# rajasekarv/vega

Hardware: AMD Instinct MI355X
Metric: rows/sec (whole node) reduce_by_key i64→i64, 1e9 rows, 1/2/4/8 GPU (higher is better)
Workload: dtype int64; 1 GPU; C1: 1e9 (i64,i64) uniform keys in [0,2^63), reduce_by_key(sum), 256 partitions (BASELINE.json configs[1]); weak scaling: --rows per GPU; rows_per_gpu=1000000000, key_bits=63, nparts=256, distinct_keys_out=1000000000

## Files before the change

vega_amd/csrc/vega_api.hip:

```cpp
#include <hip/hip_runtime.h>
#include <rccl/rccl.h>
#include <cmath>
#include <cstdio>
#include <cstring>
#include <map>
#include <string>
#include <vector>

#include "../../include/vega_common.h"
#include "../../include/vega_gpu.h"
#include "vega_internal.h"

using namespace vega;

struct RddImpl {
    uint64_t n = 0;
    int vtype = 0;
    int64_t *d_k = nullptr;
    void *d_v = nullptr;
    void *d_v2 = nullptr;
    uint64_t alloc_rows = 0;
    uint32_t nparts = 1;
    bool sorted = false;
    bool grouped = false;
// ... 1532 lines not shown
                          int64_t *out_k, int64_t *out_va, int64_t *out_vb,
                          uint64_t cap, uint64_t *h_nout, void *d_ws, size_t ws_bytes) {
    Ws ws(d_ws, ws_bytes);
    hipError_t e = join_sorted((hipStream_t)stream, ak, av, na, bk, bv, nb, order_mode,
                               out_k, out_va, out_vb, cap, h_nout, ws);
    return e == hipSuccess ? VEGA_OK : VEGA_ERR_HIP;
}

size_t vega_dev_select_ws_bytes(uint64_t num, uint64_t cand_cap) {
    return select_ws_bytes(num, cand_cap);
}

int vega_dev_select_k_i64(void *stream, const int64_t *keys, const int64_t *vals, uint64_t n,
                          uint64_t num, int descending, uint64_t cand_cap,
                          int64_t *out_k, int64_t *out_v, uint64_t *h_nout, int *h_passes,
                          void *d_ws, size_t ws_bytes) {
    if (!h_nout || !h_passes) return VEGA_ERR_INVALID;
    *h_nout = 0;
    *h_passes = 0;
    if (n >= (1ULL << 32)) return VEGA_ERR_UNSUPPORTED;
    const uint64_t m = num < n ? num : n;
    if (!m) return VEGA_OK;
    if (!keys || !vals || !out_k || !out_v) return VEGA_ERR_INVALID;
    if (!d_ws || ws_bytes < select_ws_bytes(m, cand_cap)) return VEGA_ERR_CAP;
    Ws ws(d_ws, ws_bytes);
    const char *msg = "";
    hipError_t e = select_k((hipStream_t)stream, keys, vals, n, m, descending != 0, cand_cap,
                            out_k, out_v, h_nout, h_passes, ws, &msg);
    if (e == hipSuccess) e = hipStreamSynchronize((hipStream_t)stream);
    if (e != hipSuccess && *msg) fprintf(stderr, "vega_dev_select_k_i64: %s\n", msg);
    if (e == hipErrorNotSupported) return VEGA_ERR_UNSUPPORTED;
    return e == hipSuccess ? VEGA_OK : (e == hipErrorOutOfMemory ? VEGA_ERR_CAP : VEGA_ERR_HIP);
}

int vega_dev_reduce_pairs(void *stream, const int64_t *keys, const void *vals, uint64_t n, int op,
                          int64_t *h_out_k, void *h_out_v, void *d_ws, size_t ws_bytes) {
    if (!n || !keys || !vals || !h_out_k || !h_out_v) return VEGA_ERR_INVALID;
    if (op != VEGA_OP_SUM_I64 && op != VEGA_OP_SUM_F64 && op != VEGA_OP_MIN_I64 &&
        op != VEGA_OP_MAX_I64)
        return VEGA_ERR_INVALID;
    Ws ws(d_ws, ws_bytes);
    hipError_t e = col_reduce((hipStream_t)stream, keys, vals, n, op, h_out_k, h_out_v, ws);
    if (e == hipErrorNotSupported) return VEGA_ERR_UNSUPPORTED;
    return e == hipSuccess ? VEGA_OK : (e == hipErrorOutOfMemory ? VEGA_ERR_CAP : VEGA_ERR_HIP);
}

int vega_dev_sample(void *stream, const int64_t *keys, const void *vals, uint64_t n,
                    int with_replacement, double fraction, uint64_t seed, uint64_t start,
                    int64_t *out_k, void *out_v, uint64_t cap, uint64_t *h_nout,
                    void *d_ws, size_t ws_bytes) {
    if (!h_nout) return VEGA_ERR_INVALID;
    *h_nout = 0;
    SampleSpec sp;
    int rc = sample_spec(with_replacement, fraction, seed, start, &sp, nullptr, 0);
    if (rc) return rc;
    if (n >= (1ULL << 32)) return VEGA_ERR_UNSUPPORTED;
    if (!n) return VEGA_OK;
    if (!keys || !vals) return VEGA_ERR_INVALID;
    if (!d_ws || ws_bytes < sample_ws_bytes(n)) return VEGA_ERR_NOMEM;
    Ws ws(d_ws, ws_bytes);
    SamplePlan pl;
    uint64_t total = 0;
    hipError_t e = sample_count((hipStream_t)stream, n, sp, &pl, &total, ws);
    if (e != hipSuccess) return hip_rc(e);
    *h_nout = total;
    if (total >= (1ULL << 32)) return VEGA_ERR_UNSUPPORTED;
    if (total > cap) return VEGA_ERR_CAP;
    if (!total) return VEGA_OK;
    if (!out_k || !out_v) return VEGA_ERR_INVALID;
    e = sample_emit((hipStream_t)stream, (const uint64_t *)keys, (const uint64_t *)vals, n, sp,
                    pl, (uint64_t *)out_k, (uint64_t *)out_v);
    if (e == hipSuccess) e = hipStreamSynchronize((hipStream_t)stream);
    return hip_rc(e);
}

int vega_phase_prof_read(unsigned long long out[8], int reset) {
    unsigned long long *b = vega::phase_prof_buf();
    if (!b) return VEGA_ERR_UNSUPPORTED;
    if (hipMemcpy(out, b, 8 * 8, hipMemcpyDeviceToHost) != hipSuccess) return VEGA_ERR_HIP;
    if (reset) (void)hipMemset(b, 0, 8 * 8);
    return VEGA_OK;
}

int vega_dev_checksum_pairs(void *stream, const int64_t *keys, const int64_t *vals,
                            uint64_t n, uint64_t *h_sum, void *d_ws, size_t ws_bytes) {
    Ws ws(d_ws, ws_bytes);
    return checksum_pairs((hipStream_t)stream, keys, vals, n, h_sum, ws) == hipSuccess
               ? VEGA_OK : VEGA_ERR_HIP;
}

}
```

vega_amd/csrc/vega_kernels.hip:

```cpp

#include <hip/hip_runtime.h>
#include <cmath>
#include <cstdint>
#include <cstdio>
#include <cstring>
#include <mutex>
#include <string>
#include <unordered_map>
#include <vector>

#include "../../include/vega_common.h"
#include "vega_internal.h"

#define HIP_TRY(x)                                                              \
    do {                                                                        \
        hipError_t _e = (x);                                                    \
        if (_e != hipSuccess) return _e;                                        \
    } while (0)

namespace vega {

constexpr int BLOCK = 256;
constexpr int IPT = 16;
constexpr int TILE = BLOCK * IPT;
// ... 632 lines not shown
        uint32_t chunk0 = (uint32_t)w * (64 * SIPT);
        uint32_t chunk_n = tn > chunk0 ? tn - chunk0 : 0;
#pragma unroll
        for (int r = 0; r < SIPT; ++r) {
            uint32_t local = (uint32_t)r * 64 + lane;
            if (local < chunk_n) {
                uint32_t d = dd[r];
                uint32_t pos = hist[slot * 256 + d] + whist[w * 256 + d] + rank[r];
                if (HAS_VALS) spk[pos] = make_ulonglong2(kk[r], vv[r]);
                else sk[pos] = kk[r];
            }
        }
        VEGA_PHASE_MARK(4)
    };

    auto stage_writeout = [&](int slot, uint32_t tn) {
        for (uint32_t p = t; p < tn; p += SB) {
            uint64_t k, v = 0;
            if (HAS_VALS) {
                ulonglong2 kv = spk[p];
                k = kv.x;
                v = kv.y;
            } else {
                k = sk[p];
            }
            uint32_t d = df(k);
            uint64_t gpos = (uint64_t)tilebase[slot * 256 + d] + (p - hist[slot * 256 + d]);
            if (OUT_PK) {
                ((ulonglong2 *)out_k)[gpos] = make_ulonglong2(k, v);
                if (h32_out)
                    h32_out[gpos] = (uint32_t)vega_hash_u64(k);
            } else {
                out_k[gpos] = k;
                if (HAS_VALS) out_v[gpos] = v;
                if (h32_out)
                    h32_out[gpos] = (uint32_t)vega_hash_u64(k);
            }
        }
        VEGA_PHASE_MARK(5)
    };

    for (int i = t; i < SW * 256; i += SB) whist[i] = 0;
    if (t == 0) vbp[0] = atomicAdd(ticket, 1u);
    __syncthreads();
    uint32_t vbA = vbp[0];
    if (vbA >= nblocks) return;
    int slotA = 0;
    stage_rank(vbA, 0);
    uint32_t tnA = tn_cur;
    __syncthreads();
    stage_reorder(0, tnA);
    __syncthreads();
    for (int i = t; i < SW * 256; i += SB) whist[i] = 0;
    if (t == 0) vbp[1] = atomicAdd(ticket, 1u);
    __syncthreads();

    while (true) {
        int slotB = 1 - slotA;
        uint32_t vbB = vbp[slotB];
        bool haveB = vbB < nblocks;
        uint32_t tnB = 0;
        if (haveB) {
            stage_rank(vbB, slotB);
            tnB = tn_cur;
        }
        stage_lookback(vbA, slotA, tnA);
        __syncthreads();
        VEGA_PHASE_MARK(3)
        stage_writeout(slotA, tnA);
        if (!haveB) return;
        __syncthreads();
        stage_reorder(slotB, tnB);
        __syncthreads();
        for (int i = t; i < SW * 256; i += SB) whist[i] = 0;
        if (t == 0) vbp[slotA] = atomicAdd(ticket, 1u);
        __syncthreads();
        vbA = vbB;
        tnA = tnB;
        slotA = slotB;
    }
#undef VEGA_PHASE_MARK
}

static unsigned long long *g_phase_buf = nullptr;
static int g_phase_mode = 0;
unsigned long long *phase_prof_buf() {
    static bool checked = false;
    if (!checked) {
        checked = true;
        const char *e = getenv("VEGA_PHASE_PROF");
        if (e && (e[0] == '1' || e[0] == '2')) {
            g_phase_mode = e[0] - '0';
            (void)hipMalloc(&g_phase_buf, 8 * 8);
            (void)hipMemset(g_phase_buf, 0, 8 * 8);
        }
    }
    return g_phase_buf;
}
int phase_prof_mode() { return g_phase_mode; }

template <class DF>
static hipError_t scatter_pass_osw(hipStream_t s, const uint64_t *in_k, const uint64_t *in_v,
                                   uint64_t n, const uint32_t *gbase_d,
                                   unsigned long long *desc, uint32_t *ticket,
                                   uint64_t *out_k, uint64_t *out_v, uint32_t *h32_out,
                                   int *d_abort, unsigned long long *ff, int ptag,
                                   bool has_vals, bool in_pk, bool out_pk,
                                   DF df, const char *prof_name) {
    unsigned long long *phc = phase_prof_buf();
    if (phase_prof_mode() == 2) ptag |= 0x100;
    uint32_t nb = nblocks_for(n);
    HIP_TRY(hipMemsetAsync(ff, 0,
                           ((size_t)((nb + OSW_GRP - 1) / OSW_GRP) +
                            (size_t)((nb + OSW_SUP - 1) / OSW_SUP)) * 256 * 8, s));
    HIP_TRY(hipMemsetAsync(ticket, 0, 4, s));
    ProfScope ps(prof_name, s);
    size_t sh = (has_vals ? 16 : 8) * (size_t)TILE +
                (2 * 256 + 8 * 256 + 8 + 8 + 2 * 256) * 4;
    uint32_t grid = nb < 512 ? nb : 512;
    if (!has_vals) {
        hipLaunchKernelGGL((k_scatter_osw<DF, false, false, false>), dim3(grid), dim3(512), sh, s,
                           in_k, nullptr, n, nb, gbase_d, desc, ticket, out_k, nullptr, h32_out, d_abort, ff, phc, ptag, df);
    } else if (!in_pk && !out_pk) {
        hipLaunchKernelGGL((k_scatter_osw<DF, true, false, false>), dim3(grid), dim3(512), sh, s,
                           in_k, in_v, n, nb, gbase_d, desc, ticket, out_k, out_v, h32_out, d_abort, ff, phc, ptag, df);
    } else if (!in_pk && out_pk) {
        hipLaunchKernelGGL((k_scatter_osw<DF, true, false, true>), dim3(grid), dim3(512), sh, s,
                           in_k, in_v, n, nb, gbase_d, desc, ticket, out_k, nullptr, h32_out, d_abort, ff, phc, ptag, df);
    } else if (in_pk && out_pk) {
        hipLaunchKernelGGL((k_scatter_osw<DF, true, true, true>), dim3(grid), dim3(512), sh, s,
                           in_k, nullptr, n, nb, gbase_d, desc, ticket, out_k, nullptr, h32_out, d_abort, ff, phc, ptag, df);
    } else {
        hipLaunchKernelGGL((k_scatter_osw<DF, true, true, false>), dim3(grid), dim3(512), sh, s,
                           in_k, nullptr, n, nb, gbase_d, desc, ticket, out_k, out_v, h32_out, d_abort, ff, phc, ptag, df);
    }
    return hipGetLastError();
}

template <class DF>
static hipError_t scatter_pass(hipStream_t s, const uint64_t *in_k, const uint64_t *in_v,
                               uint64_t n, uint32_t *bh, uint64_t *out_k, uint64_t *out_v,
                               bool has_vals, uint32_t ndigits, DF df, Ws &ws,
                               const char *prof_name) {
    uint32_t nb = nblocks_for(n);
    Ws w2 = ws;
    uint32_t *raw = (uint32_t *)w2.take((size_t)nb * 256 * 4);
    if (!raw) return hipErrorOutOfMemory;
    {
        ProfScope ps("hist", s);
        hipLaunchKernelGGL(k_block_hist<DF>, dim3(nb), dim3(BLOCK), 0, s, in_k, n, nb,
                           ndigits, bh, raw, df);
        HIP_TRY(hipGetLastError());
    }
    {
        ProfScope ps("scan", s);
        HIP_TRY(scan_u32_excl(s, bh, (uint64_t)ndigits * nb, w2));
    }
    {
        ProfScope ps(prof_name, s);
        size_t sh = (has_vals ? 2 : 1) * (size_t)TILE * 8 + (256 + 4 * 256 + 64) * 4;
        if (has_vals)
            hipLaunchKernelGGL((k_scatter<DF, true>), dim3(nb), dim3(BLOCK), sh, s,
                               in_k, in_v, n, nb, bh, raw, out_k, out_v, df);
        else
            hipLaunchKernelGGL((k_scatter<DF, false>), dim3(nb), dim3(BLOCK), sh, s,
                               in_k, nullptr, n, nb, bh, raw, out_k, nullptr, df);
        HIP_TRY(hipGetLastError());
    }
    return hipSuccess;
}


double bucket_rows_estimate(const uint64_t *samp, uint32_t ns, uint64_t n) {
    static thread_local uint32_t bslot[4096];
    static thread_local bool bused[4096];
    if (ns > 2048) ns = 2048;
    memset(bused, 0, sizeof bused);
// ... 178 lines not shown
            if (je == wcap && je < n && h32[je] == hh[j + 1]) {
                uint32_t slot = atomicAdd(wl_count, 1u);
                if (slot < CLEANUP_WL_CAP) wl[slot] = gi;
                else *err = 1;
                continue;
            }
            uint64_t len = je - gi;
            if (len == 1) continue;
            if (!strict && len == 2) continue;
            bool fix;
            if (strict) {
                uint64_t k0 = k[ST * gi];
                bool dirty = false;
                for (uint64_t x = gi + 1; x < je && !dirty; x++) dirty = (k[ST * x] != k0);
                fix = dirty;
            } else {
                uint32_t breaks = 0;
                uint64_t prev = k[ST * gi];
                for (uint64_t x = gi + 1; x < je && breaks < 2; x++) {
                    uint64_t cx = k[ST * x];
                    breaks += cx != prev;
                    prev = cx;
                }
                fix = breaks > 1;
            }
            if (!fix) continue;
            if (len > 64) { *err = 1; continue; }
            for (uint64_t x = gi + 1; x < je; x++) {
                uint64_t kx = k[ST * x], vx = vb[ST * x];
                uint64_t y = x;
                while (y > gi && k[ST * (y - 1)] > kx) {
                    k[ST * y] = k[ST * (y - 1)];
                    vb[ST * y] = vb[ST * (y - 1)];
                    y--;
                }
                k[ST * y] = kx;
                vb[ST * y] = vx;
            }
        }
    }
}

__global__ void k_group_cleanup_long(const uint64_t *k, const uint32_t *h32,
                                     uint64_t n, int packed, int strict, int *err,
                                     const unsigned long long *wl,
                                     const uint32_t *wl_count) {
    const int ST = packed ? 2 : 1;
    __shared__ unsigned long long s_end;
    __shared__ unsigned int s_breaks;
    uint32_t cnt = *wl_count;
    if (cnt > CLEANUP_WL_CAP) cnt = CLEANUP_WL_CAP;
    for (uint32_t e = blockIdx.x; e < cnt; e += gridDim.x) {
        uint64_t gi = wl[e];
        uint32_t h = h32[gi];
        if (threadIdx.x == 0) { s_end = n; s_breaks = 0; }
        __syncthreads();
        for (uint64_t base = gi + 1; base < s_end; base += blockDim.x) {
            uint64_t x = base + threadIdx.x;
            if (x < n && h32[x] != h) atomicMin(&s_end, (unsigned long long)x);
            __syncthreads();
        }
        uint64_t je = s_end;
        uint64_t k0 = k[ST * gi];
        for (uint64_t base = gi + 1; base < je && s_breaks < 2; base += blockDim.x) {
            uint64_t x = base + threadIdx.x;
            if (x < je) {
                bool br = strict ? (k[ST * x] != k0) : (k[ST * x] != k[ST * (x - 1)]);
                if (br) atomicAdd(&s_breaks, 1u);
            }
            __syncthreads();
        }
        if (threadIdx.x == 0) {
            bool bad = strict ? (s_breaks != 0) : (s_breaks > 1);
            if (bad) *err = 1;
        }
        __syncthreads();
    }
}

constexpr int FIN_FT = 2048, FIN_SLACK = 256, FIN_BUCKET_CAP = 256, FIN_B = 512;
constexpr int FIN_SPAN = FIN_FT + 2 * FIN_SLACK;
constexpr int FIN_LPT = FIN_SPAN / FIN_B;
constexpr int FIN_GRID = 512;
constexpr double FIN_MIN_BUCKET_ROWS = 24.0;
static_assert(FIN_SPAN % FIN_B == 0 && FIN_FT % FIN_B == 0, "whole rounds per block");
static_assert(FIN_SPAN <= 65536, "span positions are kept as u16");
static_assert(FIN_SLACK >= FIN_BUCKET_CAP, "a capped bucket must close inside the slack");
static_assert(FIN_BUCKET_CAP % 64 == 0, "a bucket is ranked in whole wave rounds");

__device__ __forceinline__ void fin_wave_sync() {
    __builtin_amdgcn_fence(__ATOMIC_ACQ_REL, "wavefront");
    __builtin_amdgcn_wave_barrier();
}

__device__ __forceinline__ uint32_t fin_wave_scan_incl(uint32_t x) {
    int v = (int)x;
    v += __builtin_amdgcn_update_dpp(0, v, 0x111, 0xf, 0xf, false);
    v += __builtin_amdgcn_update_dpp(0, v, 0x112, 0xf, 0xf, false);
    v += __builtin_amdgcn_update_dpp(0, v, 0x114, 0xf, 0xf, false);
    v += __builtin_amdgcn_update_dpp(0, v, 0x118, 0xf, 0xf, false);
    v += __builtin_amdgcn_update_dpp(0, v, 0x142, 0xa, 0xf, false);
    v += __builtin_amdgcn_update_dpp(0, v, 0x143, 0xc, 0xf, false);
    return (uint32_t)v;
}

__device__ __forceinline__ void fin_fix_run(const ulonglong2 *s_row, uint16_t *s_src,
                                            int p, int len, int *err) {
    const int pe = p + len;
    for (int x = p + 1; x < pe; x++) {
        uint16_t sx = s_src[x];
        int y = x;
        while (y > p && s_src[y - 1] > sx) {
            s_src[y] = s_src[y - 1];
            y--;
        }
        s_src[y] = sx;
    }
    if (len == 2) return;
    uint32_t breaks = 0;
    uint64_t prev = s_row[s_src[p]].x;
    for (int x = p + 1; x < pe && breaks < 2; x++) {
        uint64_t cx = s_row[s_src[x]].x;
        breaks += cx != prev;
        prev = cx;
    }
    if (breaks <= 1) return;
    if (len > 64) { *err = 1; return; }
    for (int x = p + 1; x < pe; x++) {
        uint16_t sx = s_src[x];
        uint64_t kx = s_row[sx].x;
        int y = x;
        while (y > p && s_row[s_src[y - 1]].x > kx) {
            s_src[y] = s_src[y - 1];
            y--;
        }
        s_src[y] = sx;
    }
}

__global__ __launch_bounds__(FIN_B) void k_bucket_finish(const uint64_t *in, uint64_t *out,
                                                         uint64_t n, int *err,
                                                         uint32_t *fin_heads) {
    __shared__ ulonglong2 s_row[FIN_SPAN];
    __shared__ uint32_t s_h[FIN_SPAN];
    __shared__ uint16_t s_src[FIN_SPAN];
    __shared__ uint16_t s_bk[FIN_SPAN];
    __shared__ __attribute__((aligned(16))) uint32_t s_cnt[FIN_B / 64][256];
    __shared__ int s_lo, s_hi, s_bad, s_nbk;
    __shared__ uint32_t s_heads[FIN_B / 64];

    const uint32_t ntiles = (uint32_t)((n + FIN_FT - 1) / FIN_FT);
    const int lane = threadIdx.x & 63, w = threadIdx.x >> 6;

    auto bounds = [&](uint32_t tile, uint64_t *g0, int *m) {
        const uint64_t t0 = (uint64_t)tile * FIN_FT;
        const uint64_t t1 = (n - t0 < FIN_FT) ? n : t0 + FIN_FT;
        *g0 = (t0 < FIN_SLACK) ? 0 : t0 - FIN_SLACK;
        *m = (int)(((n - t1 < FIN_SLACK) ? n : t1 + FIN_SLACK) - *g0);
    };
    ulonglong2 r[FIN_LPT];
    auto fetch = [&](uint32_t tile) {
        uint64_t g0;
        int m;
        bounds(tile, &g0, &m);
#pragma unroll
        for (int q = 0; q < FIN_LPT; ++q) {
            int li = q * FIN_B + threadIdx.x;
            r[q] = ((const ulonglong2 *)in)[g0 + (li < m ? li : m - 1)];
        }
    };

    auto order_tile = [&](uint64_t g0, int m, int a0, int a1) -> bool {
        const uint32_t bfirst = s_h[a0] >> 8, blast = s_h[a1 - 1] >> 8;
        for (int li = threadIdx.x; li < a0; li += FIN_B)
            if ((s_h[li] >> 8) != bfirst && (s_h[li + 1] >> 8) == bfirst) s_lo = li + 1;
        for (int li = a1 + threadIdx.x; li < m; li += FIN_B)
            if ((s_h[li] >> 8) != blast && (s_h[li - 1] >> 8) == blast) s_hi = li;
        __syncthreads();
        const int lo = s_lo, hi = s_hi;
        if ((lo == 0 && g0 > 0) || (hi == m && g0 + m < n)) {
            if (threadIdx.x == 0) *err = 1;
            return false;
        }
        for (int li = lo + threadIdx.x; li < hi; li += FIN_B)
            if (li == lo || (s_h[li] >> 8) != (s_h[li - 1] >> 8))
                s_bk[atomicAdd(&s_nbk, 1)] = (uint16_t)li;
        __syncthreads();

        uint32_t *cnt = s_cnt[w];
        const int nbk = s_nbk;
        int bs_next = (w < nbk) ? s_bk[w] : 0;
        for (int e = w; e < nbk; e += FIN_B / 64) {
            const int bs = bs_next;
            bs_next = (e + FIN_B / 64 < nbk) ? s_bk[e + FIN_B / 64] : 0;
            ((uint4 *)cnt)[lane] = make_uint4(0, 0, 0, 0);
            const int over = bs + FIN_BUCKET_CAP < hi ? bs + FIN_BUCKET_CAP : bs;
            const int l0 = bs + lane < hi ? bs + lane : bs;
            const uint32_t b = s_h[bs] >> 8, bover = s_h[over] >> 8, h0 = s_h[l0];
            fin_wave_sync();
            if (over != bs && bover == b) {
                if (lane == 0) s_bad = 1;
                continue;
            }
            uint32_t hh[FIN_BUCKET_CAP / 64], old[FIN_BUCKET_CAP / 64];
            bool val[FIN_BUCKET_CAP / 64];
            bool go = true;
#pragma unroll
            for (int q = 0; q < FIN_BUCKET_CAP / 64; ++q) {
                val[q] = false;
                if (go) {
                    const int li = bs + 64 * q + lane;
                    hh[q] = q == 0 ? h0 : (li < hi ? s_h[li] : 0);
                    val[q] = li < hi && (hh[q] >> 8) == b;
                    if (val[q]) old[q] = atomicAdd(&cnt[hh[q] & 0xFF], 1u);
                    go = __all(val[q]);
                }
            }
            fin_wave_sync();
            const uint4 c = ((const uint4 *)cnt)[lane];
            const uint32_t sum = c.x + c.y + c.z + c.w;
            const uint32_t ex = fin_wave_scan_incl(sum) - sum;
            ((uint4 *)cnt)[lane] = make_uint4(ex, ex + c.x, ex + c.x + c.y, ex + c.x + c.y + c.z);
            fin_wave_sync();
#pragma unroll
            for (int q = 0; q < FIN_BUCKET_CAP / 64; ++q)
                if (val[q])
                    s_src[bs + (int)(cnt[hh[q] & 0xFF] + old[q])] = (uint16_t)(bs + 64 * q + lane);
            fin_wave_sync();
            if (c.x >= 2) fin_fix_run(s_row, s_src, bs + (int)ex, (int)c.x, err);
            if (c.y >= 2) fin_fix_run(s_row, s_src, bs + (int)(ex + c.x), (int)c.y, err);
            if (c.z >= 2) fin_fix_run(s_row, s_src, bs + (int)(ex + c.x + c.y), (int)c.z, err);
            if (c.w >= 2)
                fin_fix_run(s_row, s_src, bs + (int)(ex + c.x + c.y + c.z), (int)c.w, err);
            fin_wave_sync();
        }
        __syncthreads();
        if (s_bad) {
            if (threadIdx.x == 0) *err = 1;
            return false;
        }
        return true;
    };

    uint32_t tile = blockIdx.x;
    if (tile < ntiles) fetch(tile);
    while (tile < ntiles) {
        const uint64_t t0 = (uint64_t)tile * FIN_FT;
        const uint64_t t1 = (n - t0 < FIN_FT) ? n : t0 + FIN_FT;
        uint64_t g0;
        int m;
        bounds(tile, &g0, &m);
        const int a0 = (int)(t0 - g0), a1 = (int)(t1 - g0);
        if (threadIdx.x == 0) { s_lo = 0; s_hi = m; s_bad = 0; s_nbk = 0; }
#pragma unroll
        for (int q = 0; q < FIN_LPT; ++q) {
            int li = q * FIN_B + threadIdx.x;
            if (li < m) {
                s_row[li] = r[q];
                s_h[li] = (uint32_t)vega_hash_u64(r[q].x);
            }
        }
        __syncthreads();
        const uint32_t next = tile + gridDim.x;
        if (next < ntiles) fetch(next);
        const bool done = order_tile(g0, m, a0, a1);
        if (done) {
            const int lo = s_lo;
            uint32_t heads = 0;
            uint16_t si[FIN_FT / FIN_B], sp[FIN_FT / FIN_B];
#pragma unroll
            for (int q = 0; q < FIN_FT / FIN_B; ++q) {
                const int p = a0 + q * FIN_B + threadIdx.x;
                const int pc = p < a1 ? p : a1 - 1;
                si[q] = s_src[pc];
                sp[q] = s_src[pc > lo ? pc - 1 : pc];
            }
            ulonglong2 row[FIN_FT / FIN_B];
            uint64_t pkey[FIN_FT / FIN_B];
#pragma unroll
            for (int q = 0; q < FIN_FT / FIN_B; ++q) {
                row[q] = s_row[si[q]];
                pkey[q] = s_row[sp[q]].x;
            }
#pragma unroll
            for (int q = 0; q < FIN_FT / FIN_B; ++q) {
                const int p = a0 + q * FIN_B + threadIdx.x;
                if (p < a1) ((ulonglong2 *)out)[g0 + p] = row[q];
                const bool head = p < a1 && (p == lo || row[q].x != pkey[q]);
                heads += (uint32_t)__popcll(__ballot(head));
            }
            if (lane == 0) s_heads[w] = heads;
        }
        __syncthreads();
        if (done && threadIdx.x == 0) {
            uint32_t t = 0;
#pragma unroll
            for (int i = 0; i < FIN_B / 64; ++i) t += s_heads[i];
            fin_heads[tile] = t;
        }
        tile = next;
    }
}

__global__ void k_unpack_rows(const uint64_t *pk, uint64_t n, uint64_t *k, uint64_t *v) {
    uint64_t stride = (uint64_t)gridDim.x * blockDim.x;
    for (uint64_t i = (uint64_t)blockIdx.x * blockDim.x + threadIdx.x; i < n; i += stride) {
        ulonglong2 r = ((const ulonglong2 *)pk)[i];
        k[i] = r.x;
        v[i] = r.y;
    }
}

hipError_t group_sort_u64(hipStream_t s, const uint64_t *in_k, const uint64_t *in_v,
                          uint64_t n, int force_hbytes, int *order_tag,
                          int want_packed, int *out_packed, Ws &ws,
                          const uint64_t **res_k, const uint64_t **res_v,
                          int route, int *route_taken, const uint32_t **fin_heads) {
    *res_k = in_k;
    *res_v = in_v;
    if (out_packed) *out_packed = 0;
    if (order_tag) *order_tag = 0;
    if (route_taken) *route_taken = 0;
    if (fin_heads) *fin_heads = nullptr;
    if (n <= 1) return hipSuccess;
    if (n >= (1ULL << 32)) return hipErrorNotSupported;
    uint32_t nb = nblocks_for(n);

    uint64_t *pA = (uint64_t *)ws.take(n * 16);
    uint64_t *pB = (uint64_t *)ws.take(n * 16);
    unsigned long long *desc = (unsigned long long *)ws.take((size_t)256 * nb * 8);
    uint32_t *gbase_d = (uint32_t *)ws.take(8 * 256 * 4);
    uint32_t *ticket = (uint32_t *)ws.take(256);
    uint32_t *h8 = (uint32_t *)ws.take(8 * 256 * 4);
    int *d_err = (int *)ws.take(256);
    int *d_abort = (int *)ws.take(256);
    unsigned long long *ff_d = (unsigned long long *)ws.take(
        ((size_t)((nb + OSW_GRP - 1) / OSW_GRP) +
         (size_t)((nb + OSW_SUP - 1) / OSW_SUP)) * 256 * 8);
    uint32_t *h32buf = (uint32_t *)ws.take(n * 4);
    unsigned long long *wl = (unsigned long long *)ws.take(CLEANUP_WL_CAP * 8);
    uint32_t *wl_count = (uint32_t *)ws.take(256);
    uint32_t *fh_d = (uint32_t *)ws.take(((size_t)2 * nb + 1) * 4);
    if (!pA || !pB || !desc || !gbase_d || !ticket || !h8 || !d_err || !d_abort ||
        !ff_d || !h32buf || !wl || !wl_count || !fh_d)
        return hipErrorOutOfMemory;
    HIP_TRY(hipMemsetAsync(d_abort, 0, 4, s));
    HIP_TRY(hipMemsetAsync(desc, 0, (size_t)nb * 256 * 8, s));
    int ptag_ctr = 0;
    const int strict = (force_hbytes != 0 || order_tag != nullptr) ? 1 : 0;

    static thread_local uint32_t hh[8 * 256];
    static thread_local uint32_t gb_host[8 * 256];
    bool pass_on[8] = {true, true, true, true, true, true, true, true};

    auto exact_hists = [&](bool hashsrc, int nbl, int *active) -> hipError_t {
        HIP_TRY(hipMemsetAsync(h8, 0, 8 * 256 * 4, s));
        {
            ProfScope ps(hashsrc ? "ghist" : "hist8", s);
            uint32_t gb = nb < 2048 ? nb : 2048;
            if (hashsrc && nbl == 4)
                hipLaunchKernelGGL((k_hist8t<true, 4>), dim3(gb), dim3(BLOCK), 0, s, in_k, n, h8);
            else if (hashsrc)
                hipLaunchKernelGGL((k_hist8t<true, 5>), dim3(gb), dim3(BLOCK), 0, s, in_k, n, h8);
            else
                hipLaunchKernelGGL((k_hist8t<false, 8>), dim3(gb), dim3(BLOCK), 0, s, in_k, n, h8);
            HIP_TRY(hipGetLastError());
        }
        HIP_TRY(hipMemcpyAsync(hh, h8, 8 * 256 * 4, hipMemcpyDeviceToHost, s));
        HIP_TRY(hipStreamSynchronize(s));
        *active = 0;
        for (int p = 0; p < 8; ++p) {
            int nz = 0;
            uint32_t running = 0;
            for (int d = 0; d < 256; ++d) {
                nz += hh[p * 256 + d] != 0;
                gb_host[p * 256 + d] = running;
                running += hh[p * 256 + d];
            }
            pass_on[p] = nz > 1;
            *active += pass_on[p];
        }
        return hipMemcpyAsync(gbase_d, gb_host, 8 * 256 * 4, hipMemcpyHostToDevice, s);
    };

    auto run_key_passes = [&](const uint64_t **rk, const uint64_t **rv) -> hipError_t {
        int plist[8], np = 0;
        for (int p = 0; p < 8; ++p)
            if (pass_on[p]) plist[np++] = p;
        if (np == 0) { *rk = in_k; *rv = in_v; return hipSuccess; }
        const uint64_t *cur = nullptr;
        for (int i = 0; i < np; ++i) {
            int p = plist[i];
            bool in_pk = i > 0, out_pk = i < np - 1;
            uint64_t *dbuf = ((i & 1) == 0) ? pA : pB;
            uint64_t *dk = dbuf;
            uint64_t *dv = out_pk ? nullptr : dbuf + n;
            RadixDigit df{8 * p};
            HIP_TRY(scatter_pass_osw(s, i == 0 ? in_k : cur, i == 0 ? in_v : nullptr,
                                     n, gbase_d + p * 256, desc, ticket,
                                     dk, dv, nullptr, d_abort, ff_d, ptag_ctr++, true, in_pk, out_pk, df, "radix_scatter"));
            cur = dk;
        }
        *rk = cur;
        *rv = cur + n;
        return hipSuccess;
    };

    int a_est = 8;
    bool samp_repeat = false;
    double bucket_rows = 0;
    HIP_TRY(sample_active_passes(s, in_k, n, ws, &a_est, &samp_repeat, &bucket_rows));

    const uint64_t *cur_k = in_k, *cur_v = in_v;
    if (a_est <= 5 && route == 0) {
        int active = 8;
        HIP_TRY(exact_hists(false, 8, &active));
        if (active <= 5) {
            HIP_TRY(run_key_passes(res_k, res_v));
            int ab = 0;
            HIP_TRY(hipMemcpyAsync(&ab, d_abort, 4, hipMemcpyDeviceToHost, s));
            HIP_TRY(hipStreamSynchronize(s));
            return ab ? hipErrorUnknown : hipSuccess;
        }
    }

    const int hbytes = force_hbytes ? force_hbytes : ((n <= (1ULL << 30)) ? 4 : 5);
    int active5 = 0;
    HIP_TRY(exact_hists(true, hbytes, &active5));
    const bool keep_pk = want_packed != 0;
    if (!strict && hbytes == 4 && keep_pk && route != 1 &&
        (route == 2 || (!samp_repeat && bucket_rows >= FIN_MIN_BUCKET_ROWS))) {
        for (int i = 1; i < 4; ++i) {
            uint64_t *dk = (i & 1) ? pA : pB;
            HashByteDigit df{8 * i};
            HIP_TRY(scatter_pass_osw(s, i == 1 ? in_k : cur_k, i == 1 ? in_v : nullptr,
                                     n, gbase_d + i * 256, desc, ticket, dk, nullptr, nullptr,
                                     d_abort, ff_d, ptag_ctr++, true, i > 1, true, df, "radix_scatter"));
            cur_k = dk;
        }
        HIP_TRY(hipMemsetAsync(d_err, 0, 4, s));
        {
            ProfScope ps("group_cleanup", s);
            ProfScope pk("bucket_finish", s);
            const uint32_t ntiles = (uint32_t)((n + FIN_FT - 1) / FIN_FT);
            hipLaunchKernelGGL(k_bucket_finish, dim3(ntiles < FIN_GRID ? ntiles : FIN_GRID),
                               dim3(FIN_B), 0, s, cur_k, pB, n, d_err, fh_d);
            HIP_TRY(hipGetLastError());
        }
        int fl[2] = {0, 0};
        HIP_TRY(hipMemcpyAsync(&fl[0], d_err, 4, hipMemcpyDeviceToHost, s));
        HIP_TRY(hipMemcpyAsync(&fl[1], d_abort, 4, hipMemcpyDeviceToHost, s));
        HIP_TRY(hipStreamSynchronize(s));
        if (fl[1]) return hipErrorUnknown;
        if (!fl[0]) {
            if (out_packed) *out_packed = 1;
            if (route_taken) *route_taken = 2;
            if (fin_heads) *fin_heads = fh_d;
            *res_k = pB;
            *res_v = nullptr;
            return hipSuccess;
        }
        cur_k = in_k;
        cur_v = in_v;
    }
    if (route_taken) *route_taken = 1;
    for (int i = 0; i < hbytes; ++i) {
        bool in_pk = i > 0, out_pk = keep_pk || (i < hbytes - 1);
        bool last = i == hbytes - 1;
        uint64_t *dbuf = ((i & 1) == 0) ? pA : pB;
        uint64_t *dk = dbuf;
        uint64_t *dv = out_pk ? nullptr : dbuf + n;
        HashByteDigit df{8 * i};
        HIP_TRY(scatter_pass_osw(s, i == 0 ? in_k : cur_k, i == 0 ? in_v : nullptr,
                                 n, gbase_d + i * 256, desc, ticket,
                                 dk, dv, last ? h32buf : nullptr,
                                 d_abort, ff_d, ptag_ctr++, true, in_pk, out_pk, df, "radix_scatter"));
        cur_k = dk;
        cur_v = out_pk ? nullptr : dk + n;
    }
    HIP_TRY(hipMemsetAsync(d_err, 0, 4, s));
    HIP_TRY(hipMemsetAsync(wl_count, 0, 4, s));
    {
        ProfScope ps("group_cleanup", s);
        uint32_t gb = nb < 2048 ? nb : 2048;
        hipLaunchKernelGGL(k_group_cleanup, dim3(gb), dim3(BLOCK), 0, s,
                           (uint64_t *)cur_k, (uint64_t *)cur_v, h32buf, n,
                           keep_pk ? 1 : 0, strict, d_err, wl, wl_count);
        HIP_TRY(hipGetLastError());
        hipLaunchKernelGGL(k_group_cleanup_long, dim3(512), dim3(BLOCK), 0, s,
                           cur_k, h32buf, n, keep_pk ? 1 : 0, strict, d_err, wl, wl_count);
        HIP_TRY(hipGetLastError());
    }
    int flags[2] = {0, 0};
    HIP_TRY(hipMemcpyAsync(&flags[0], d_err, 4, hipMemcpyDeviceToHost, s));
    HIP_TRY(hipMemcpyAsync(&flags[1], d_abort, 4, hipMemcpyDeviceToHost, s));
    HIP_TRY(hipStreamSynchronize(s));
    if (flags[1]) return hipErrorUnknown;
    int err = flags[0];
    if (err) {
        int active = 8;
        HIP_TRY(exact_hists(false, 8, &active));
        HIP_TRY(run_key_passes(&cur_k, &cur_v));
        int ab2 = 0;
        HIP_TRY(hipMemcpyAsync(&ab2, d_abort, 4, hipMemcpyDeviceToHost, s));
        HIP_TRY(hipStreamSynchronize(s));
        if (ab2) return hipErrorUnknown;
    } else if (keep_pk && out_packed) {
        *out_packed = 1;
    }
    if (order_tag && !err) *order_tag = (hbytes == 4) ? 4 : 0;
    *res_k = cur_k;
    *res_v = cur_v;
    return hipSuccess;
}


template <bool PK>
__global__ void k_head_count(const uint64_t *k, uint64_t n, uint32_t *hc) {
    __shared__ uint32_t wsum[BLOCK / 64];
    uint64_t tbase = (uint64_t)blockIdx.x * TILE;
    uint32_t c = 0;
#pragma unroll
    for (int j = 0; j < IPT; ++j) {
        uint64_t idx = tbase + (uint64_t)j * BLOCK + threadIdx.x;
        if (idx < n)
            c += (idx == 0) || (k[PK ? 2 * idx : idx] != k[PK ? 2 * (idx - 1) : idx - 1]);
    }
    for (int off = 32; off > 0; off >>= 1) c += __shfl_down(c, off);
    int lane = threadIdx.x & 63, w = threadIdx.x >> 6;
// ... 1979 lines not shown
```

Baseline: 20.56 billion rows/s.

## Rank fine buckets block-wide in grouped 16-bit counters instead of per-wave loops

Rewrites the bucket-finish ordering step. The old code ranked each bucket on one wave at a time with a per-wave 256-bin counter. The new code finds bucket heads with ballots and a chunk scan, ranks up to 56 buckets at once in shared 16-bit packed counters, and special-cases runs of two or three equal-hash rows with a small closed-form ordering. It also drops the s_h and s_bk shared arrays in favour of registers, and adds an optional templated phase profiler that writes into an enlarged profiling buffer. The aim is more parallelism and fewer serial wave iterations in the finishing kernel; the cost is more block-wide barriers and more complex indexing.

```diff
diff --git a/vega_amd/csrc/vega_api.hip b/vega_amd/csrc/vega_api.hip
--- a/vega_amd/csrc/vega_api.hip
+++ b/vega_amd/csrc/vega_api.hip
@@ -1638,6 +1638,14 @@
     return VEGA_OK;
 }
 
+int vega_fin_phase_prof_read(unsigned long long out[8], int reset) {
+    unsigned long long *b = vega::phase_prof_buf();
+    if (!b) return VEGA_ERR_UNSUPPORTED;
+    if (hipMemcpy(out, b + 8, 8 * 8, hipMemcpyDeviceToHost) != hipSuccess) return VEGA_ERR_HIP;
+    if (reset) (void)hipMemset(b + 8, 0, 8 * 8);
+    return VEGA_OK;
+}
+
 int vega_dev_checksum_pairs(void *stream, const int64_t *keys, const int64_t *vals,
                             uint64_t n, uint64_t *h_sum, void *d_ws, size_t ws_bytes) {
     Ws ws(d_ws, ws_bytes);
diff --git a/vega_amd/csrc/vega_kernels.hip b/vega_amd/csrc/vega_kernels.hip
--- a/vega_amd/csrc/vega_kernels.hip
+++ b/vega_amd/csrc/vega_kernels.hip
@@ -738,6 +738,7 @@
 #undef VEGA_PHASE_MARK
 }
 
+constexpr int PHASE_SLOTS = 16;
 static unsigned long long *g_phase_buf = nullptr;
 static int g_phase_mode = 0;
 unsigned long long *phase_prof_buf() {
@@ -747,8 +748,8 @@
         const char *e = getenv("VEGA_PHASE_PROF");
         if (e && (e[0] == '1' || e[0] == '2')) {
             g_phase_mode = e[0] - '0';
-            (void)hipMalloc(&g_phase_buf, 8 * 8);
-            (void)hipMemset(g_phase_buf, 0, 8 * 8);
+            (void)hipMalloc(&g_phase_buf, PHASE_SLOTS * 8);
+            (void)hipMemset(g_phase_buf, 0, PHASE_SLOTS * 8);
         }
     }
     return g_phase_buf;
@@ -1093,16 +1094,15 @@
 constexpr int FIN_SPAN = FIN_FT + 2 * FIN_SLACK;
 constexpr int FIN_LPT = FIN_SPAN / FIN_B;
 constexpr int FIN_GRID = 512;
+constexpr int FIN_CHUNKS = FIN_SPAN / 64;
+constexpr int FIN_GROUP = 56;
+constexpr int FIN_CSTRIDE = 260;
 constexpr double FIN_MIN_BUCKET_ROWS = 24.0;
+constexpr int FIN_PHASE0 = 8, FIN_PHASES = 8;
 static_assert(FIN_SPAN % FIN_B == 0 && FIN_FT % FIN_B == 0, "whole rounds per block");
 static_assert(FIN_SPAN <= 65536, "span positions are kept as u16");
 static_assert(FIN_SLACK >= FIN_BUCKET_CAP, "a capped bucket must close inside the slack");
 static_assert(FIN_BUCKET_CAP % 64 == 0, "a bucket is ranked in whole wave rounds");
-
-__device__ __forceinline__ void fin_wave_sync() {
-    __builtin_amdgcn_fence(__ATOMIC_ACQ_REL, "wavefront");
-    __builtin_amdgcn_wave_barrier();
-}
 
 __device__ __forceinline__ uint32_t fin_wave_scan_incl(uint32_t x) {
     int v = (int)x;
@@ -1149,19 +1149,31 @@
     }
 }
 
+template <bool PROF>
 __global__ __launch_bounds__(FIN_B) void k_bucket_finish(const uint64_t *in, uint64_t *out,
                                                          uint64_t n, int *err,
-                                                         uint32_t *fin_heads) {
+                                                         uint32_t *fin_heads,
+                                                         unsigned long long *phc) {
     __shared__ ulonglong2 s_row[FIN_SPAN];
-    __shared__ uint32_t s_h[FIN_SPAN];
     __shared__ uint16_t s_src[FIN_SPAN];
-    __shared__ uint16_t s_bk[FIN_SPAN];
-    __shared__ __attribute__((aligned(16))) uint32_t s_cnt[FIN_B / 64][256];
-    __shared__ int s_lo, s_hi, s_bad, s_nbk;
+    __shared__ uint16_t s_bstart[FIN_SPAN + 2];
+    __shared__ __attribute__((aligned(16))) uint32_t s_cnt[FIN_GROUP * FIN_CSTRIDE / 2];
+    __shared__ uint32_t s_edge[FIN_CHUNKS];
+    __shared__ uint32_t s_tot[FIN_CHUNKS];
+    __shared__ int s_of, s_ol, s_bad;
     __shared__ uint32_t s_heads[FIN_B / 64];
+    uint16_t *const s_cnt16 = (uint16_t *)s_cnt;
 
     const uint32_t ntiles = (uint32_t)((n + FIN_FT - 1) / FIN_FT);
     const int lane = threadIdx.x & 63, w = threadIdx.x >> 6;
+    unsigned long long tprev = PROF ? __builtin_amdgcn_s_memtime() : 0;
+    unsigned long long pacc[FIN_PHASES] = {};
+#define VEGA_PHASE_MARK(i)                                                     \
+    if (PROF) {                                                                \
+        unsigned long long tnow = __builtin_amdgcn_s_memtime();                \
+        pacc[i] += tnow - tprev;                                               \
+        tprev = tnow;                                                          \
+    }
 
     auto bounds = [&](uint32_t tile, uint64_t *g0, int *m) {
         const uint64_t t0 = (uint64_t)tile * FIN_FT;
@@ -1170,7 +1182,9 @@
         *m = (int)(((n - t1 < FIN_SLACK) ? n : t1 + FIN_SLACK) - *g0);
     };
     ulonglong2 r[FIN_LPT];
-    auto fetch = [&](uint32_t tile) {
+    uint32_t h[FIN_LPT];
+    int lo_out = 0;
+    auto fetch =[&](uint32_t tile) {
         uint64_t g0;
         int m;
         bounds(tile, &g0, &m);
@@ -1182,74 +1196,149 @@
     };
 
     auto order_tile = [&](uint64_t g0, int m, int a0, int a1) -> bool {
-        const uint32_t bfirst = s_h[a0] >> 8, blast = s_h[a1 - 1] >> 8;
-        for (int li = threadIdx.x; li < a0; li += FIN_B)
-            if ((s_h[li] >> 8) != bfirst && (s_h[li + 1] >> 8) == bfirst) s_lo = li + 1;
-        for (int li = a1 + threadIdx.x; li < m; li += FIN_B)
-            if ((s_h[li] >> 8) != blast && (s_h[li - 1] >> 8) == blast) s_hi = li;
+        uint32_t inc[FIN_LPT], ishead = 0;
+#pragma unroll
+        for (int q = 0; q < FIN_LPT; ++q) {
+            const int li = q * FIN_B + threadIdx.x, c = q * (FIN_B / 64) + w;
+            const uint32_t bk = h[q] >> 8;
+            uint32_t pb = (uint32_t)__shfl_up((int)bk, 1);
+            if (lane == 0) pb = c ? s_edge[c - 1] : ~0u;
+            const bool head = li < m && (li == 0 || bk != pb);
+            ishead |= (uint32_t)head << q;
+            const uint64_t heads = __ballot(head);
+            inc[q] = (uint32_t)__popcll(heads & (~0ull >> (63 - lane)));
+            if (lane == 0) s_tot[c] = (uint32_t)__popcll(heads);
+        }
+        for (int i = threadIdx.x; i < FIN_GROUP * FIN_CSTRIDE / 8; i += FIN_B)
+            ((uint4 *)s_cnt)[i] = make_uint4(0, 0, 0, 0);
         __syncthreads();
-        const int lo = s_lo, hi = s_hi;
+        const uint32_t tot = lane < FIN_CHUNKS ? s_tot[lane] : 0;
+        const uint32_t tinc = fin_wave_scan_incl(tot);
+        int ord[FIN_LPT];
+#pragma unroll
+        for (int q = 0; q < FIN_LPT; ++q) {
+            const int li = q * FIN_B + threadIdx.x, c = q * (FIN_B / 64) + w;
+            ord[q] = (int)(__shfl((int)(tinc - tot), c) + inc[q]) - 1;
+            if (ishead >> q & 1) s_bstart[ord[q]] = (uint16_t)li;
+            if (li == a0) s_of = ord[q];
+            if (li == a1 - 1) s_ol = ord[q];
+        }
+        const int nb = __shfl((int)tinc, FIN_CHUNKS - 1);
+        if (threadIdx.x == 0) s_bstart[nb] = (uint16_t)m;
+        __syncthreads();
+        VEGA_PHASE_MARK(1)
+        const int of = s_of, nbk = s_ol - of + 1;
+        const int lo = s_bstart[of], hi = s_bstart[of + nbk];
+        lo_out = lo;
         if ((lo == 0 && g0 > 0) || (hi == m && g0 + m < n)) {
             if (threadIdx.x == 0) *err = 1;
             return false;
         }
-        for (int li = lo + threadIdx.x; li < hi; li += FIN_B)
-            if (li == lo || (s_h[li] >> 8) != (s_h[li - 1] >> 8))
-                s_bk[atomicAdd(&s_nbk, 1)] = (uint16_t)li;
+
+        int bs[FIN_LPT], rel[FIN_LPT];
+        bool act[FIN_LPT];
+#pragma unroll
+        for (int q = 0; q < FIN_LPT; ++q) {
+            const int li = q * FIN_B + threadIdx.x;
+            act[q] = li >= lo && li < hi;
+            rel[q] = ord[q] - of;
+            bs[q] = act[q] ? s_bstart[ord[q]] : 0;
+            if (act[q] && li - bs[q] >= FIN_BUCKET_CAP) s_bad = 1;
+        }
+        for (int gb = 0; gb < nbk; gb += FIN_GROUP) {
+            if (gb) {
+                for (int i = threadIdx.x; i < FIN_GROUP * FIN_CSTRIDE / 8; i += FIN_B)
+                    ((uint4 *)s_cnt)[i] = make_uint4(0, 0, 0, 0);
+                __syncthreads();
+            }
+            const int ng = nbk - gb < FIN_GROUP ? nbk - gb : FIN_GROUP;
+            bool in[FIN_LPT];
+            int ci[FIN_LPT], old[FIN_LPT];
+#pragma unroll
+            for (int q = 0; q < FIN_LPT; ++q) {
+                in[q] = act[q] && (unsigned)(rel[q] - gb) < (unsigned)FIN_GROUP;
+                ci[q] = in[q] ? (rel[q] - gb) * FIN_CSTRIDE + (int)(h[q] & 0xFF) : 0;
+                const int sh = (ci[q] & 1) * 16;
+                if (in[q]) old[q] = (int)((atomicAdd(&s_cnt[ci[q] >> 1], 1u << sh) >> sh) & 0xFFFF);
+            }
+            __syncthreads();
+            VEGA_PHASE_MARK(2)
+            if (s_bad) {
+                if (threadIdx.x == 0) *err = 1;
+                return false;
+            }
+            for (int e = w; e < ng; e += 2 * (FIN_B / 64)) {
+                const bool two = e + FIN_B / 64 < ng;
+                const int ee[2] = {e, two ? e + FIN_B / 64 : e};
+                uint2 c[2];
+#pragma unroll
+                for (int j = 0; j < 2; ++j)
+                    c[j] = ((const uint2 *)(s_cnt + ee[j] * (FIN_CSTRIDE / 2)))[lane];
+#pragma unroll
+                for (int j = 0; j < 2; ++j) {
+                    const uint32_t c0 = c[j].x & 0xFFFF, c1 = c[j].x >> 16;
+                    const uint32_t c2 = c[j].y & 0xFFFF, c3 = c[j].y >> 16;
+                    const uint32_t sum = c0 + c1 + c2 + c3;
+                    const uint32_t inc = fin_wave_scan_incl(sum), ex = inc - sum;
+                    if (j == 0 || two) {
+                        ((uint2 *)(s_cnt + ee[j] * (FIN_CSTRIDE / 2)))[lane] =
+                            make_uint2(ex | (ex + c0) << 16, (ex + c0 + c1) | (ex + c0 + c1 + c2) << 16);
+                        if (lane == 63) s_cnt16[ee[j] * FIN_CSTRIDE + 256] = (uint16_t)inc;
+                    }
+                }
+            }
+            __syncthreads();
+            VEGA_PHASE_MARK(3)
+            int p0[FIN_LPT], cn[FIN_LPT];
+#pragma unroll
+            for (int q = 0; q < FIN_LPT; ++q) {
+                cn[q] = 0;
+                if (in[q]) {
+                    const int off = s_cnt16[ci[q]];
+                    cn[q] = s_cnt16[ci[q] + 1] - off;
+                    p0[q] = bs[q] + off;
+                    s_src[p0[q] + old[q]] = (uint16_t)(q * FIN_B + threadIdx.x);
+                }
+            }
+            __syncthreads();
+            VEGA_PHASE_MARK(6)
+            uint32_t oth[FIN_LPT];
+#pragma unroll
+            for (int q = 0; q < FIN_LPT; ++q) {
+                oth[q] = 0;
+                if (cn[q] == 2) {
+                    oth[q] = s_src[p0[q] + 1 - old[q]];
+                } else if (cn[q] == 3) {
+                    const int s1 = old[q] == 2 ? 0 : old[q] + 1, s2 = old[q] == 0 ? 2 : old[q] - 1;
+                    oth[q] = (uint32_t)s_src[p0[q] + s1] | (uint32_t)s_src[p0[q] + s2] << 16;
+                }
+            }
+            __syncthreads();
+#pragma unroll
+            for (int q = 0; q < FIN_LPT; ++q) {
+                const int li = q * FIN_B + threadIdx.x;
+                const int o1 = (int)(oth[q] & 0xFFFF), o2 = (int)(oth[q] >> 16);
+                if (cn[q] == 2) {
+                    const int slot = li > o1;
+                    if (slot != old[q]) s_src[p0[q] + slot] = (uint16_t)li;
+                } else if (cn[q] == 3) {
+                    const uint64_t k0 = s_row[li].x, k1 = s_row[o1].x, k2 = s_row[o2].x;
+                    const int rin = (o1 < li) + (o2 < li);
+                    const int r1 = (li < o1) + (o2 < o1);
+                    const bool dirty = rin == 1 ? (k1 != k0 && k2 != k0)
+                                     : r1 == 1 ? (k0 != k1 && k2 != k1)
+                                               : (k0 != k2 && k1 != k2);
+                    const int rkey = (k1 < k0 || (k1 == k0 && o1 < li)) +
+                                     (k2 < k0 || (k2 == k0 && o2 < li));
+                    const int slot = dirty ? rkey : rin;
+                    if (slot != old[q]) s_src[p0[q] + slot] = (uint16_t)li;
+                } else if (cn[q] > 3 && old[q] == 0) {
+                    fin_fix_run(s_row, s_src, p0[q], cn[q], err);
+                }
+            }
+        }
         __syncthreads();
-
-        uint32_t *cnt = s_cnt[w];
-        const int nbk = s_nbk;
-        int bs_next = (w < nbk) ? s_bk[w] : 0;
-        for (int e = w; e < nbk; e += FIN_B / 64) {
-            const int bs = bs_next;
-            bs_next = (e + FIN_B / 64 < nbk) ? s_bk[e + FIN_B / 64] : 0;
-            ((uint4 *)cnt)[lane] = make_uint4(0, 0, 0, 0);
-            const int over = bs + FIN_BUCKET_CAP < hi ? bs + FIN_BUCKET_CAP : bs;
-            const int l0 = bs + lane < hi ? bs + lane : bs;
-            const uint32_t b = s_h[bs] >> 8, bover = s_h[over] >> 8, h0 = s_h[l0];
-            fin_wave_sync();
-            if (over != bs && bover == b) {
-                if (lane == 0) s_bad = 1;
-                continue;
-            }
-            uint32_t hh[FIN_BUCKET_CAP / 64], old[FIN_BUCKET_CAP / 64];
-            bool val[FIN_BUCKET_CAP / 64];
-            bool go = true;
-#pragma unroll
-            for (int q = 0; q < FIN_BUCKET_CAP / 64; ++q) {
-                val[q] = false;
-                if (go) {
-                    const int li = bs + 64 * q + lane;
-                    hh[q] = q == 0 ? h0 : (li < hi ? s_h[li] : 0);
-                    val[q] = li < hi && (hh[q] >> 8) == b;
-                    if (val[q]) old[q] = atomicAdd(&cnt[hh[q] & 0xFF], 1u);
-                    go = __all(val[q]);
-                }
-            }
-            fin_wave_sync();
-            const uint4 c = ((const uint4 *)cnt)[lane];
-            const uint32_t sum = c.x + c.y + c.z + c.w;
-            const uint32_t ex = fin_wave_scan_incl(sum) - sum;
-            ((uint4 *)cnt)[lane] = make_uint4(ex, ex + c.x, ex + c.x + c.y, ex + c.x + c.y + c.z);
-            fin_wave_sync();
-#pragma unroll
-            for (int q = 0; q < FIN_BUCKET_CAP / 64; ++q)
-                if (val[q])
-                    s_src[bs + (int)(cnt[hh[q] & 0xFF] + old[q])] = (uint16_t)(bs + 64 * q + lane);
-            fin_wave_sync();
-            if (c.x >= 2) fin_fix_run(s_row, s_src, bs + (int)ex, (int)c.x, err);
-            if (c.y >= 2) fin_fix_run(s_row, s_src, bs + (int)(ex + c.x), (int)c.y, err);
-            if (c.z >= 2) fin_fix_run(s_row, s_src, bs + (int)(ex + c.x + c.y), (int)c.z, err);
-            if (c.w >= 2)
-                fin_fix_run(s_row, s_src, bs + (int)(ex + c.x + c.y + c.z), (int)c.w, err);
-            fin_wave_sync();
-        }
-        __syncthreads();
-        if (s_bad) {
-            if (threadIdx.x == 0) *err = 1;
-            return false;
-        }
+        VEGA_PHASE_MARK(7)
         return true;
     };
 
@@ -1262,21 +1351,21 @@
         int m;
         bounds(tile, &g0, &m);
         const int a0 = (int)(t0 - g0), a1 = (int)(t1 - g0);
-        if (threadIdx.x == 0) { s_lo = 0; s_hi = m; s_bad = 0; s_nbk = 0; }
+        if (threadIdx.x == 0) s_bad = 0;
 #pragma unroll
         for (int q = 0; q < FIN_LPT; ++q) {
             int li = q * FIN_B + threadIdx.x;
-            if (li < m) {
-                s_row[li] = r[q];
-                s_h[li] = (uint32_t)vega_hash_u64(r[q].x);
-            }
+            h[q] = (uint32_t)vega_hash_u64(r[q].x);
+            if (li < m) s_row[li] = r[q];
+            if (lane == 63) s_edge[q * (FIN_B / 64) + w] = h[q] >> 8;
         }
         __syncthreads();
+        VEGA_PHASE_MARK(0)
         const uint32_t next = tile + gridDim.x;
         if (next < ntiles) fetch(next);
         const bool done = order_tile(g0, m, a0, a1);
         if (done) {
-            const int lo = s_lo;
+            const int lo = lo_out;
             uint32_t heads = 0;
             uint16_t si[FIN_FT / FIN_B], sp[FIN_FT / FIN_B];
 #pragma unroll
@@ -1302,6 +1391,7 @@
             }
             if (lane == 0) s_heads[w] = heads;
         }
+        VEGA_PHASE_MARK(4)
         __syncthreads();
         if (done && threadIdx.x == 0) {
             uint32_t t = 0;
@@ -1309,8 +1399,12 @@
             for (int i = 0; i < FIN_B / 64; ++i) t += s_heads[i];
             fin_heads[tile] = t;
         }
+        VEGA_PHASE_MARK(5)
         tile = next;
     }
+    if (PROF && lane == 0)
+        for (int i = 0; i < FIN_PHASES; ++i) atomicAdd(&phc[FIN_PHASE0 + i], pacc[i]);
+#undef VEGA_PHASE_MARK
 }
 
 __global__ void k_unpack_rows(const uint64_t *pk, uint64_t n, uint64_t *k, uint64_t *v) {
@@ -1454,8 +1548,14 @@
             ProfScope ps("group_cleanup", s);
             ProfScope pk("bucket_finish", s);
             const uint32_t ntiles = (uint32_t)((n + FIN_FT - 1) / FIN_FT);
-            hipLaunchKernelGGL(k_bucket_finish, dim3(ntiles < FIN_GRID ? ntiles : FIN_GRID),
-                               dim3(FIN_B), 0, s, cur_k, pB, n, d_err, fh_d);
+            unsigned long long *phc = phase_prof_buf();
+            const dim3 grid(ntiles < FIN_GRID ? ntiles : FIN_GRID);
+            if (phc)
+                hipLaunchKernelGGL(k_bucket_finish<true>, grid, dim3(FIN_B), 0, s, cur_k, pB, n,
+                                   d_err, fh_d, phc);
+            else
+                hipLaunchKernelGGL(k_bucket_finish<false>, grid, dim3(FIN_B), 0, s, cur_k, pB, n,
+                                   d_err, fh_d, nullptr);
             HIP_TRY(hipGetLastError());
         }
         int fl[2] = {0, 0};
```

Result: faster. 22.33 billion rows/s (median of 6 runs) (+8.6%).
